# UBC-AWP/vision-sam3-yolo-lameless

Hardware: AMD Instinct MI355X
Metric: frames/sec (whole node) for YOLO+SAM3+DINOv3 feature extraction, 1080p clips (higher is better)
Workload: dtype f16; 1 GPU; BASELINE cfg#5, dense schedule: fused per-frame path on a synthetic 5 s @ 30 fps 1080p clip (150 unique BGR frames resident in HBM): YOLOv8-l detect (letterbox 384x640, NMS, scale_boxes; f16 plan) -> SAM (Hiera-B+ image encoder + FPN at 1024x1024, box-prompted mask decoder, 1080p mask + statistics + contour features) + DINOv3 ViT-L/16 embed (224x224) on EVERY frame; per-frame records packed, gathe; parallelism=one clip per GPU, 1 GPU(s), one gather per step, streams=7

## Files before the change

### include/lmx.h

```cpp
#ifndef LMX_H
#define LMX_H
#include <stdint.h>
#ifdef __cplusplus
extern "C" {
#endif

#define LMX_VERSION 100

#define LMX_OK 0
#define LMX_EINVAL (-1)
#define LMX_EHIP (-2)

typedef void* lmx_stream_t;

int lmx_version(void);
const char* lmx_last_error(void);
int lmx_device_count(void);

enum { LMX_F16 = 0, LMX_F32 = 1 };
enum { LMX_ACT_NONE = 0, LMX_ACT_SILU = 1, LMX_ACT_GELU = 2 , LMX_ACT_RELU = 3,
       LMX_ACT_SWIGLU = 4  };

typedef struct {
  const void* A;
// ... 166 lines not shown
enum { LMX_HIERA_MLP_IMG = 0, LMX_HIERA_MLP_FUSED = 1, LMX_HIERA_MLP_LAUNCHES = 2 };
typedef struct {
  int32_t H, W, Hf, Ho, Wo, Hfo, join, attn, ln1, shortcut, query, window, ln_out, mlp, emit_ln1, stage_end, keep, x16, join_out, clone;
} lmx_hiera_block_t;
int lmx_h_hiera_blocks(const lmx_hiera_config_t* config, int* n_blocks_host);
int lmx_h_hiera_plan_rows(const lmx_hiera_config_t* config, int n, const int* rows_in_host, int lowest, lmx_hiera_block_t* records_host);
int lmx_h_hiera_plan(const lmx_hiera_config_t* config, int n, int nh, int nw, int lowest, lmx_hiera_block_t* records_host, int* rows_host);

int lmx_k_add_bcast(const void* a, int a_dtype, int64_t lda, const float* b, int64_t ldb, int b_rows, void* out,
                    int out_dtype, int64_t ldo, int64_t rows, int D, lmx_stream_t stream);
int lmx_k_prompt_box(const float* boxes, int64_t ldb, float* sparse, int n, double sx, double sy, float S,
                     const float* gauss, const float* corner, int F, lmx_stream_t stream);
int lmx_k_hyper_mask(const void* up, const float* hyper, float* logits, int n, int G, int C, lmx_stream_t stream);
int lmx_k_mask_post(const float* logits, int n, int L, int T, int nh, int nw, int h, int w, uint8_t* mask,
                    int64_t* stats, float* workspace, lmx_stream_t stream);
int lmx_k_prompt_points(const float* points, const int32_t* labels, int Np, const float* boxes, int64_t ldb, float* sparse, int n,
                        double sx, double sy, float S, const float* gauss, const float* point_embed, const float* not_a_point,
                        const float* corner, int F, lmx_stream_t stream);
#define LMX_MASK_EMBED_PARAMS 4684
int lmx_k_mask_embed(const float* mask_input, const void* emb, int emb_dtype, int64_t lde, const float* params, float* keys,
                     int64_t ldk, int n, int G, lmx_stream_t stream);
int lmx_k_hyper_mask_multi(const void* up, const float* hyper, float* logits, int n, int M, int G, int C, lmx_stream_t stream);
int lmx_k_hyper_mask_multi_f32(const float* up, const float* hyper, float* logits, int n, int M, int G, int C, int act,
                               lmx_stream_t stream);
int lmx_k_mask_logits(const float* logits, int n, int L, int T, int nh, int nw, int h, int w, float* out, lmx_stream_t stream);

int lmx_k_mask_score(const float* logits, int n, int L, int T, int nh, int nw, int h, int w, double thr, double off,
                     const int32_t* idx, int64_t* out, lmx_stream_t stream);
int lmx_k_nms_boxes(const float* boxes, int64_t ldb, const float* scores, const uint8_t* valid, int n, double iou, int32_t* keep_out,
                    int32_t* count_out, void* workspace, lmx_stream_t stream);
// ... 1 lines not shown
enum { LMX_RECORD_MAX_FIELDS = 16, LMX_RECORD_MAX_MAPS = 4 };
typedef struct { const void* src; int64_t row_bytes, offset; int32_t map, n_src; } lmx_record_field_t;
int lmx_k_pack_records(const lmx_record_field_t* fields_host, int n_fields, const int32_t* const* row_maps_host, int n_maps, int64_t n_valid,
                       int64_t n_rows, int64_t stride, uint8_t* out, lmx_stream_t stream);

enum { LMX_REC_U8 = 0, LMX_REC_I32 = 1, LMX_REC_I64 = 2, LMX_REC_F32 = 3 };
enum { LMX_STREAMS_LANES = 0, LMX_STREAMS_RR = 1 };
typedef struct { char name[16]; int32_t dtype, ndim; int64_t shape[2], offset, nbytes; } lmx_record_field_layout_t;
typedef struct { int32_t n_fields, reserved; int64_t stride; lmx_record_field_layout_t fields[LMX_RECORD_MAX_FIELDS]; } lmx_record_layout_t;
int lmx_h_record_layout(int h, int w, int hidden, int max_det, int scheduled, lmx_record_layout_t* out_host);
int lmx_h_stream_plan(int n_chunks, int max_streams, int layout, int* pool_host, int* det_host, int* emb_host, int32_t* sam_host);
int lmx_h_row_map(int n, const int32_t* idx_host, int n_idx, const char* what, int32_t* map_host, int32_t* ran_host);

int64_t lmx_contour_workspace_bytes(int n, int h, int w);
int lmx_k_contour_features(const uint8_t* mask, int n, int h, int w, int64_t* out, void* workspace, lmx_stream_t stream);

int lmx_h_mask_features(const uint8_t* mask_host, int h, int w, double* out_host);

int lmx_h_iou_matrix(const double* a, int n, const double* b, int m, double* out);
int lmx_h_assign(const double* cost, int n, int m, int* row_to_col, int* col_to_row);

enum { LMX_FILT_BILINEAR = 2, LMX_FILT_BICUBIC = 3 };
int lmx_h_pil_tables(int in_size, int out_size, int filt, int32_t* bounds_host, int32_t* kk_host, int64_t cap, int* ksize_host);
int lmx_h_aa_tables(int in_size, int out_size, int filt, int32_t* bounds_host, float* kk_host, int64_t cap, int* ksize_host);
int lmx_h_identity_table(int n, int32_t* bounds_host, int32_t* kk_host);
int lmx_h_segment_cols(const int32_t* bounds_host, int n_out, int tile);

typedef struct lmx_dino lmx_dino;
enum { LMX_DINO_V2 = 0, LMX_DINO_V3 = 1 };
enum { LMX_RECIPE_PIL = 0, LMX_RECIPE_FLOAT = 1 };
// ... 216 lines not shown
```

### vision-sam3-yolo-lameless_amd/csrc/contour.hip

```cpp
#include "common.h"

namespace {

typedef unsigned long long u64;

__device__ __forceinline__ int pc(u64 v) { return __builtin_popcountll(v); }
__device__ __forceinline__ int ld(const int* p) { return __hip_atomic_load(p, __ATOMIC_RELAXED, __HIP_MEMORY_SCOPE_AGENT); }

__device__ __forceinline__ int uf_find(const int* L, int i) {
  int p = ld(L + i);
  while (p != i) {
    i = p;
    p = ld(L + i);
  }
  return i;
}

__device__ __forceinline__ void uf_union(int* L, int a, int b) {
  for (;;) {
    a = uf_find(L, a);
    b = uf_find(L, b);
    if (a == b) return;
    if (a > b) {
      const int t = a;
// ... 89 lines not shown
      cnt[wi] = c;
    }
    __syncthreads();
    int before = 0, all = 0;
#pragma unroll
    for (int i = 0; i < WPI; ++i) {
      const int c = cnt[i];
      before += i < wi ? c : 0;
      all += c;
    }
    if (leader && k < wpr) ws.wpre[ri * wpr + k] = running + before;
    running += all;
    __syncthreads();
  }
  if (threadIdx.x == 0) ws.rowbase[ri] = running;
}

__global__ __launch_bounds__(256) void run_scan_kernel(Ws ws) {
  __shared__ int part[256];
  const int img = blockIdx.x;
  int* rb = ws.rowbase + (int64_t)img * ws.h;
  int running = 2;
  for (int y0 = 0; y0 < ws.h; y0 += 256) {
    const int y = y0 + threadIdx.x;
    const int c = y < ws.h ? (rb[y] + 1) & ~1 : 0;
    part[threadIdx.x] = c;
    __syncthreads();
    for (int o = 1; o < 256; o <<= 1) {
      const int v = threadIdx.x >= o ? part[threadIdx.x - o] : 0;
      __syncthreads();
// ... 294 lines not shown
    off += bytes;
    return p;
  };
  ws.bits = reinterpret_cast<u64*>(take(words * 8));
  ws.area2 = reinterpret_cast<long long*>(take(slots * 8));
  ws.steps = reinterpret_cast<u64*>(take(slots * 8));
  ws.best = reinterpret_cast<u64*>(take((int64_t)n * 8));
  ws.box = reinterpret_cast<int*>(take(slots * 16));
  ws.L = reinterpret_cast<int*>(take((int64_t)n * ws.cap * 4));
  ws.wpre = reinterpret_cast<int*>(take(words * 4));
  ws.rowbase = reinterpret_cast<int*>(take((int64_t)n * h * 4));
  ws.count = reinterpret_cast<int*>(take((int64_t)n * 4));
  return off;
}

}

extern "C" int64_t lmx_contour_workspace_bytes(int n, int h, int w) {
  if (n <= 0 || h <= 0 || w <= 0) return 0;
  Ws ws;
  return ws_layout(ws, nullptr, n, h, w);
}

extern "C" int lmx_k_contour_features(const uint8_t* mask, int n, int h, int w, int64_t* out, void* workspace, lmx_stream_t stream) {
  LMX_REQUIRE(mask && out && workspace, "lmx_k_contour_features: null pointer");
  LMX_REQUIRE(n > 0 && h > 1 && w > 1 && (int64_t)h * w <= 0x1fffff && (int64_t)n * h < 0x7fffffffll && n <= 65535,
              "lmx_k_contour_features: n=%d h=%d w=%d (at most 2^21 - 1 pixels per mask)", n, h, w);
  LMX_REQUIRE(aligned16(workspace), "lmx_k_contour_features: workspace alignment");
  hipStream_t st = reinterpret_cast<hipStream_t>(stream);
  const int64_t npix = (int64_t)h * w;
  Ws ws;
  ws_layout(ws, reinterpret_cast<char*>(workspace), n, h, w);
  const unsigned rows = (unsigned)((int64_t)n * h), words = grid_for((int64_t)n * h * ws.wpr);
  if (w % 4 == 0 && (reinterpret_cast<uintptr_t>(mask) & 3) == 0)
    hipLaunchKernelGGL(run_bits_kernel<true>, dim3(rows), dim3(256), 0, st, mask, ws, npix);
  else
    hipLaunchKernelGGL(run_bits_kernel<false>, dim3(rows), dim3(256), 0, st, mask, ws, npix);
  hipLaunchKernelGGL(run_scan_kernel, dim3(n), dim3(256), 0, st, ws);
  hipLaunchKernelGGL(run_init_kernel, dim3(words), dim3(256), 0, st, ws, n);
  hipLaunchKernelGGL(run_union_kernel, dim3(words), dim3(256), 0, st, ws, n);
  hipLaunchKernelGGL(run_compress_kernel, dim3(words), dim3(256), 0, st, ws, n);
  hipLaunchKernelGGL(run_sum_kernel, dim3(words), dim3(256), 0, st, ws, n);
  hipLaunchKernelGGL(run_select_kernel, dim3(words), dim3(256), 0, st, ws, n);
  hipLaunchKernelGGL(contour_final_kernel, dim3((n + 63) / 64), dim3(64), 0, st, ws, reinterpret_cast<long long*>(out), n);
  return lmx_launch_check("contour_final_kernel");
}
```

### vision-sam3-yolo-lameless_amd/csrc/sam.hip

```cpp
#include "common.h"
#include "hiera_bands.h"

namespace {

inline int grid_for(int64_t total, int block = 256) {
  int64_t g = (total + block - 1) / block;
  if (g > 256 * 8) g = 256 * 8;
  if (g < 1) g = 1;
  return (int)g;
}

constexpr int P7_T = 64;
constexpr int P7_ROW = (4 * P7_T + 3) * 3;
constexpr int P7_NDW = (P7_ROW + 3 + 3) / 4 + 1;
constexpr int P7_LOADS = (7 * P7_NDW + 255) / 256;
__global__ __launch_bounds__(256) void im2col_p7_kernel(const uint8_t* __restrict__ img, const float* __restrict__ lut,
                                                        half_t* __restrict__ out, int n, int rh, int rw, int OH, int OW, int64_t ldo) {
  __shared__ half_t lut_s[768];
  __shared__ half_t st[7 * P7_ROW];
  for (int i = threadIdx.x; i < 768; i += blockDim.x) lut_s[i] = (half_t)lut[i];
  __syncthreads();
  const int tid = threadIdx.x;
  const int chunks = (int)(ldo / 8);
  const int tpp = 256 / chunks;
// ... 334 lines not shown
      maxy = red_b[k][3] > maxy ? red_b[k][3] : maxy;
    }
    if (area) {
      unsigned long long* st = stats + (int64_t)b * 8;
      atomicAdd(&st[0], area);
      atomicAdd(&st[1], sumx);
      atomicAdd(&st[2], sumy);
      atomicMin(reinterpret_cast<long long*>(&st[3]), (long long)minx);
      atomicMin(reinterpret_cast<long long*>(&st[4]), (long long)miny);
      atomicMax(reinterpret_cast<long long*>(&st[5]), (long long)maxx);
      atomicMax(reinterpret_cast<long long*>(&st[6]), (long long)maxy);
    }
  }
}

__global__ __launch_bounds__(256) void pack_bits_kernel(const uint8_t* __restrict__ src, int64_t rows, int w, int wb,
                                                        uint8_t* __restrict__ dst) {
  const int64_t total = rows * wb;
  const bool fast = (w & 7) == 0 && ((reinterpret_cast<uintptr_t>(src) & 7) == 0);
  for (int64_t i = (int64_t)blockIdx.x * blockDim.x + threadIdx.x; i < total; i += (int64_t)gridDim.x * blockDim.x) {
    const int64_t r = i / wb;
    const int c = (int)(i - r * wb);
    const uint8_t* sp = src + r * w + (int64_t)c * 8;
    unsigned long long x = 0;
    if (fast) {
      x = *reinterpret_cast<const unsigned long long*>(sp);
    } else {
      for (int e = 0; e < 8; ++e)
        if (c * 8 + e < w) x |= (unsigned long long)sp[e] << (8 * e);
    }
// ... 205 lines not shown
  else if (dbg == 5) LMX_MASK_VARIANT(5, 5)
  else if (dbg == 8) LMX_MASK_VARIANT(1, 8)
  else if (dbg == 6) LMX_MASK_VARIANT(1, 6)
  else if (dbg == 7) LMX_MASK_VARIANT(1, 7)
  else if (dbg == 1) LMX_MASK_VARIANT(1, 1)
  else if (dbg == 9) LMX_MASK_VARIANT(1, 9)
  else LMX_MASK_VARIANT(0, 0)
#undef LMX_MASK_VARIANT
#else
  hipLaunchKernelGGL(mask_mid_kernel<0>, dim3(gmid), dim3(256), 0, st, logits, workspace, n, L, T, nh, nw, su);
  hipLaunchKernelGGL(mask_post_kernel<0>, dim3(gx, n), dim3(256), 0, st, workspace, n, nh, nw, h, w, mask, su, gmid);
#endif
  return lmx_launch_check("mask_post_kernel");
}

extern "C" int lmx_k_pack_bits(const uint8_t* src, int64_t rows, int w, uint8_t* dst, lmx_stream_t stream) {
  LMX_REQUIRE(src && dst, "lmx_k_pack_bits: null pointer");
  LMX_REQUIRE(rows > 0 && w > 0, "lmx_k_pack_bits: rows=%lld w=%d", (long long)rows, w);
  const int wb = (w + 7) / 8;
  hipLaunchKernelGGL(pack_bits_kernel, dim3(grid_for(rows * wb)), dim3(256), 0, reinterpret_cast<hipStream_t>(stream), src, rows, w, wb, dst);
  return lmx_launch_check("pack_bits_kernel");
}
```

### vision-sam3-yolo-lameless_amd/csrc/sam_model.hip

```cpp
#include <math.h>
#include <string.h>

#include <map>
#include <string>
#include <tuple>
#include <vector>

#include "model_handle.h"
#include "sam_hiera_model.h"
#include "sam_image.h"
#include "sam_lanes.h"

namespace {

const int64_t MAX_BUFFER_BYTES = 0x7fffffffll;
const int DD = LMX_SAM_DEC_D, DH = LMX_SAM_DEC_HEADS, DT = LMX_SAM_OUT_TOKENS + 2;

struct Lin {
  const void* w = nullptr;
  const float *b = nullptr, *s = nullptr;
  int N = 0, K = 0;
};

struct Norm {
// ... 698 lines not shown
    LMX_TRY(upscale(W, v, nP));
    LMX_TRY(operand(queries + DD, (int64_t)T * DD, nullptr, 0, P.qc16, n, &mask_tok));
    LMX_TRY(ffn(W.hyp, mask_tok, P.hyper));
    if (exact)
      LMX_TRY(lmx_k_hyper_mask_multi_f32(static_cast<const float*>(P.u2), P.hyper, logits, n, 1, G, 32, LMX_ACT_GELU, st));
    else
      LMX_TRY(lmx_k_hyper_mask_multi(P.u2, P.hyper, logits, n, 1, G, 32, st));
    return ffn(W.iou, iou_tok, P.iou4);
  }
};

int decode_chunk(const lmx_sam* m, const Prepared& P, int precision, const void* emb, int n, int h, int w, const float* boxes, int64_t ldb, uint8_t* mask,
                 uint8_t* mask_bits, int64_t* stats, int64_t* contour, float* iou, float* lowres, hipStream_t st) {
  const LmxSamCfg& c = m->cfg;
  const int L = 4 * c.grid();
  uint8_t* mk = mask ? mask : P.mask;
  float* logits = lowres ? lowres : P.logits;
  LMX_TRY(lmx_k_prompt_box(boxes, ldb, P.sparse, n, (double)P.nw / (double)w, (double)P.nh / (double)h, (float)c.image, m->gauss, m->corner, DD / 2, st));
  LMX_HIP(hipMemcpy2DAsync(P.tokens + LMX_SAM_OUT_TOKENS * DD, (size_t)DT * DD * 4, P.sparse, (size_t)2 * DD * 4, (size_t)2 * DD * 4, (size_t)n,
                           hipMemcpyDeviceToDevice, st));
  LMX_TRY((Dec{m, P, n, precision == LMX_SAM_EXACT, st}.lowres(emb, logits)));
  LMX_TRY(lmx_k_mask_post(logits, n, L, c.image, P.nh, P.nw, h, w, mk, stats, P.post, st));
  LMX_HIP(hipMemcpy2DAsync(iou, 4, P.iou4, 16, 4, (size_t)n, hipMemcpyDeviceToDevice, st));
  if (mask_bits) LMX_TRY(lmx_k_pack_bits(mk, (int64_t)n * h, w, mask_bits, st));
  if (contour) LMX_TRY(lmx_k_contour_features(mk, n, h, w, contour, P.contour_ws, st));
  return LMX_OK;
}

int check_call(const lmx_sam* m, const char* fn, int n, int h, int w, int precision) {
  LMX_TRY(lmx_handle_on_device(m, fn));
  LMX_REQUIRE(n > 0, "%s: n = %d frames", fn, n);
  LMX_REQUIRE(h > 0 && w > 0, "%s: frame size %d x %d", fn, h, w);
  return check_precision(m, fn, precision);
}

int check_decode(const lmx_sam* m, const char* fn, const void* in, const char* in_name, int n, int h, int w, const void* boxes, int precision,
                 const void* stats, const void* contour, const void* iou) {
  LMX_TRY(check_call(m, fn, n, h, w, precision));
  LMX_REQUIRE(in != nullptr, "%s: null pointer (%s)", fn, in_name);
  LMX_REQUIRE(boxes != nullptr, "%s: null pointer (boxes)", fn);
// ... 175 lines not shown
```

### vision-sam3-yolo-lameless_amd/lmx/_lib.py

```python
import ctypes as C
import os

_HERE = os.path.dirname(os.path.abspath(__file__))
LIB_PATH = os.environ.get("LMX_LIB") or os.path.join(_HERE, "liblmx.so")


class LmxError(RuntimeError):
    pass


class GemmDesc(C.Structure):
    _fields_ = [
        ("A", C.c_void_p), ("W", C.c_void_p), ("bias", C.c_void_p), ("scale", C.c_void_p), ("res", C.c_void_p),
        ("C", C.c_void_p),
        ("lda", C.c_int64), ("ldc", C.c_int64), ("ldr", C.c_int64),
        ("M", C.c_int32), ("N", C.c_int32), ("K", C.c_int32),
        ("act", C.c_int32), ("out_dtype", C.c_int32), ("a_mode", C.c_int32),
        ("H", C.c_int32), ("W_", C.c_int32), ("Cin", C.c_int32), ("conv_stride", C.c_int32),
        ("Ho", C.c_int32), ("Wo", C.c_int32), ("res_rows", C.c_int32), ("a_rep", C.c_int32), ("split_k", C.c_int32), ("split_stride", C.c_int64),
        ("ln_out", C.c_void_p), ("ln_gamma", C.c_void_p), ("ln_beta", C.c_void_p), ("ld_ln", C.c_int64), ("ln_eps", C.c_float),
    ]


class DinoInfo(C.Structure):
# ... 196 lines not shown
    "lmx_k_im2col_u8": (_I, [_VP, _VP, _VP, _I, _I, _I, _I, _I, _I, _I, _I, _I, _I64, _VP]),
    "lmx_k_maxpool2": (_I, [_VP, _I64, _VP, _I64, _I, _I, _I, _I, _I, _VP]),
    "lmx_k_cast_f32_f16": (_I, [_VP, _I64, _VP, _I64, _I64, _I, _VP]),
    "lmx_h_hiera_band": (_I, [C.POINTER(C.c_int), C.POINTER(C.c_int), _I, _I, _I, _I, C.POINTER(C.c_int)]),
    "lmx_h_hiera_bands": (_I, [C.POINTER(C.c_int), C.POINTER(C.c_int), _I, _I, _I, _I, C.POINTER(C.c_int)]),
    "lmx_k_band_join": (_I, [_VP, _VP, _VP, _I, _I, _I, _I, _I, _I, _VP]),
    "lmx_h_hiera_blocks": (_I, [C.POINTER(HieraConfig), C.POINTER(C.c_int)]),
    "lmx_h_hiera_plan_rows": (_I, [C.POINTER(HieraConfig), _I, C.POINTER(C.c_int), _I, C.POINTER(HieraBlock)]),
    "lmx_h_hiera_plan": (_I, [C.POINTER(HieraConfig), _I, _I, _I, _I, C.POINTER(HieraBlock), C.POINTER(C.c_int)]),
    "lmx_k_add_bcast":(_I, [_VP, _I, _I64, _VP, _I64, _I, _VP, _I, _I64, _I64, _I, _VP]),
    "lmx_h_mask_features": (_I, [_VP, _I, _I, _VP]),
    "lmx_h_iou_matrix": (_I, [_VP, _I, _VP, _I, _VP]),
    "lmx_h_assign": (_I, [_VP, _I, _I, _VP, _VP]),
    "lmx_contour_workspace_bytes": (_I64, [_I, _I, _I]),
    "lmx_k_contour_features": (_I, [_VP, _I, _I, _I, _VP, _VP, _VP]),
    "lmx_k_prompt_box": (_I, [_VP, _I64, _VP, _I, _D, _D, _F, _VP, _VP, _I, _VP]),
    "lmx_k_hyper_mask": (_I, [_VP, _VP, _VP, _I, _I, _I, _VP]),
    "lmx_k_mask_post": (_I, [_VP, _I, _I, _I, _I, _I, _I, _I, _VP, _VP, _VP, _VP]),
    "lmx_k_prompt_points": (_I, [_VP, _VP, _I, _VP, _I64, _VP, _I, _D, _D, _F, _VP, _VP, _VP, _VP, _I, _VP]),
    "lmx_k_mask_embed": (_I, [_VP, _VP, _I, _I64, _VP, _VP, _I64, _I, _I, _VP]),
    "lmx_k_hyper_mask_multi": (_I, [_VP, _VP, _VP, _I, _I, _I, _I, _VP]),
    "lmx_k_hyper_mask_multi_f32": (_I, [_VP, _VP, _VP, _I, _I, _I, _I, _I, _VP]),
    "lmx_k_mask_logits": (_I, [_VP, _I, _I, _I, _I, _I, _I, _I, _VP, _VP]),
    "lmx_k_mask_score": (_I, [_VP, _I, _I, _I, _I, _I, _I, _I, _D, _D, _VP, _VP, _VP]),
    "lmx_k_nms_boxes": (_I, [_VP, _I64, _VP, _VP, _I, _D, _VP, _VP, _VP, _VP]),
    "lmx_h_pil_tables": (_I, [_I, _I, _I, _VP, _VP, _I64, C.POINTER(C.c_int)]),
    "lmx_h_aa_tables": (_I, [_I, _I, _I, _VP, _VP, _I64, C.POINTER(C.c_int)]),
    "lmx_h_identity_table": (_I, [_I, _VP, _VP]),
    "lmx_h_segment_cols": (_I, [_VP, _I, _I]),
    "lmx_dino_image_check_host": (_I, [C.c_char_p, C.POINTER(DinoInfo)]),
# ... 111 lines not shown
```

### vision-sam3-yolo-lameless_amd/lmx/kernels.py

```python
import ctypes as C
import os
import threading

import torch

from . import _lib
from ._lib import AttnDesc, GemmDesc, LmxError, check

F16, F32 = 0, 1
ACT_NONE, ACT_SILU, ACT_GELU, ACT_RELU, ACT_SWIGLU = 0, 1, 2, 3, 4
_DT = {torch.float16: F16, torch.float32: F32}


_tls = threading.local()


def _stream(dev):
    _tls.dev = dev
    return C.c_void_p(torch.cuda.current_stream(dev).cuda_stream)


def _ptr(t):
    return C.c_void_p(t.data_ptr()) if t is not None else C.c_void_p(0)

# ... 1554 lines not shown
    check(_lib.load().lmx_k_hyper_mask(_ptr(up), _ptr(hyper), _ptr(logits), n, G, C_, _stream(dev)), "lmx_k_hyper_mask")
    return logits


def mask_post(logits, T, nh, nw, h, w):
    dev = _dev(logits)
    n, L, _ = logits.shape
    mask = torch.empty((n, h, w), dtype=torch.uint8, device=logits.device)
    stats = torch.empty((n, 8), dtype=torch.int64, device=logits.device)
    ws = torch.empty((n, nh, nw), dtype=torch.float32, device=logits.device)
    check(_lib.load().lmx_k_mask_post(_ptr(logits), n, L, T, nh, nw, h, w, _ptr(mask), _ptr(stats), _ptr(ws), _stream(dev)),
          "lmx_k_mask_post")
    return mask, stats


def prompt_points(points, labels, boxes, sx, sy, S, gauss, point_embed, not_a_point, corner):
    dev = _dev(points, labels, boxes, gauss)
    Np = 0 if points is None else points.shape[1]
    if Np:
        if (points.dtype != torch.float32 or labels.dtype != torch.int32 or not points.is_contiguous() or not labels.is_contiguous()
                or points.dim() != 3 or points.shape[2] != 2 or tuple(labels.shape) != tuple(points.shape[:2])):
            raise LmxError("prompt_points: points must be contiguous f32 [n,Np,2], labels contiguous int32 [n,Np]")
    if boxes is not None and (boxes.dtype != torch.float32 or boxes.dim() != 2 or boxes.shape[1] < 4 or boxes.stride(1) != 1):
        raise LmxError("prompt_points: boxes must be f32 [n,>=4] rows")
    n = points.shape[0] if Np else boxes.shape[0]
    if boxes is not None and boxes.shape[0] != n:
        raise LmxError("prompt_points: points and boxes disagree on n")
    Fq = gauss.shape[1]
    ldb = 0 if boxes is None else (boxes.stride(0) if n > 1 else boxes.shape[1])
    out = torch.empty((n, Np + (2 if boxes is not None else 1), 2 * Fq), dtype=torch.float32, device=dev)
# ... 95 lines not shown
    ws = torch.empty((n * 5,), dtype=torch.float32, device=boxes.device)
    check(_lib.load().lmx_k_nms_boxes(_ptr(boxes), ldb, _ptr(scores), _ptr(valid), n, float(iou), _ptr(keep), _ptr(count), _ptr(ws),
                                      _stream(dev)), "lmx_k_nms_boxes")
    return keep, count


def contour_features(mask):
    dev = _dev(mask)
    if mask.dtype != torch.uint8 or mask.dim() != 3 or not mask.is_contiguous():
        raise LmxError("contour_features: mask must be contiguous uint8 [n,h,w]")
    n, h, w = mask.shape
    lib = _lib.load()
    ws = torch.empty((int(lib.lmx_contour_workspace_bytes(n, h, w)),), dtype=torch.uint8, device=mask.device)
    out = torch.empty((n, 8), dtype=torch.int64, device=mask.device)
    check(lib.lmx_k_contour_features(_ptr(mask), n, h, w, _ptr(out), _ptr(ws), _stream(dev)), "lmx_k_contour_features")
    return out


LAUNCH_TRACE = None
_raw_lib = None
RIDGE_FLOP_PER_BYTE = 2500e12 / 8e12


def _work(name, args):
    if name == "lmx_k_gemm":
        d = args[0]._obj
        M, N, Kd = d.M, d.N, d.K
        osz = 4 if d.out_dtype == F32 else 2
        a_bytes = 2 * M * (Kd // max(d.a_rep, 1))
        if d.a_mode == 1:
# ... 109 lines not shown
```

### vision-sam3-yolo-lameless_amd/lmx/pipeline.py

```python
import os

import torch

from . import dino, sam, sam_decoder, yolo
from . import kernels as K

DATA = os.path.join(os.path.dirname(os.path.abspath(__file__)), "data")


def stream_plan(n_chunks, max_streams=4, layout="lanes"):
    if layout not in ("lanes", "rr"):
        raise ValueError(f"stream layout {layout!r}: expected 'lanes' or 'rr'")
    k = max(3, min(2 + n_chunks, int(max_streams)))
    if layout == "rr":
        return k, 0, 1, [(2 + j) % k for j in range(n_chunks)]
    return k, 0, 1, [2 + j % (k - 2) for j in range(n_chunks)]


class FusedExtractor:
    def __init__(self, device="cuda", yolo_scale="l", weight_seeds=(7, 5, 3), yolo_bn=None):
        from . import weights

        self.device = torch.device(device)
        self.serial = bool(os.environ.get("LMX_SERIAL"))
# ... 51 lines not shown
            out["ran_det"].index_fill_(0, di, 1)
            if keep_byte_masks:
                out["mask"] = torch.zeros((n, h, w), dtype=torch.uint8, device=dev)
                out["mask"].index_copy_(0, di, part["mask"])
        if ei.numel():
            out["embedding"].index_copy_(0, ei, part["embedding"])
            out["ran_emb"].index_fill_(0, ei, 1)
        return out

    def _step_dense(self, frames, conf, sam_chunk, keep_byte_masks, emb_frames=None, precision=None):
        n, h, w, _ = frames.shape
        emb_frames = frames if emb_frames is None else emb_frames
        rhw = sam.resize_longest_side(h, w, self.sam.cfg.image)
        main = torch.cuda.current_stream(self.device)
        chunks = list(range(0, n, sam_chunk))
        if self.serial:
            det_stream, emb_stream, sam_streams = main, main, [main] * len(chunks)
        else:
            n_pool, di, ei, si = stream_plan(max(1, len(chunks)), self.max_streams, self.stream_layout)
            pool = self._streams(n_pool)
            det_stream, emb_stream, sam_streams = pool[di], pool[ei], [pool[j] for j in si][:len(chunks)]
            for st in pool:
                st.wait_stream(main)
        empty = n == 0
        with torch.cuda.stream(det_stream):
            if empty:
                z = torch.zeros
                boxes, scores, cls, counts = (z((0, 300, 4), device=self.device), z((0, 300), device=self.device),
                                              z((0, 300), dtype=torch.int32, device=self.device), z((0,), dtype=torch.int32, device=self.device))
            else:
                boxes, scores, cls, src, counts = self.yolo.detect(frames, conf=conf, precision=precision)
            det_done = torch.cuda.Event()
            det_done.record(det_stream)
        with torch.cuda.stream(emb_stream):
            emb = (self.dino.embed_frames(emb_frames) if emb_frames.shape[0]
                   else torch.zeros((0, self.dino.cfg.hidden), dtype=torch.float32, device=self.device))
        masks, stats, ious, conts = [], [], [], []
        for i, st in zip(chunks, sam_streams):
            with torch.cuda.stream(st):
                enc = self.sam.encode(frames[i:i + sam_chunk], precision=precision, outputs="embedding")
                e2 = enc["fpn"][2]
                st.wait_event(det_done)
                d = self.decoder.predict(e2.view(-1, e2.shape[-1]), boxes[i:i + sam_chunk, 0, :], (h, w), rhw, precision=precision)
                conts.append(K.contour_features(d["mask"]))
            masks.append(d["mask"])
            stats.append(d["stats"])
            ious.append(d["iou"])
        for st in set(sam_streams + [det_stream, emb_stream]):
            if st is not main:
                main.wait_stream(st)
        if empty:
            mask = torch.zeros((0, h, w), dtype=torch.uint8, device=self.device)
            out = dict(boxes=boxes, scores=scores, cls=cls, counts=counts, embedding=emb,
                       mask_bits=torch.zeros((0, h, (w + 7) // 8), dtype=torch.uint8, device=self.device),
                       mask_stats=torch.zeros((0, 8), dtype=torch.int64, device=self.device),
                       mask_contour=torch.zeros((0, 8), dtype=torch.int64, device=self.device),
                       mask_iou=torch.zeros((0,), dtype=torch.float32, device=self.device))
        else:
            cat = (lambda ts: ts[0] if len(ts) == 1 else torch.cat(ts, 0))
            mask = cat(masks)
            out = dict(boxes=boxes, scores=scores, cls=cls, counts=counts, embedding=emb, mask_bits=K.pack_bits(mask),
                       mask_stats=cat(stats), mask_contour=cat(conts), mask_iou=cat(ious))
        if keep_byte_masks:
            out["mask"] = mask
        return out
```

### vision-sam3-yolo-lameless_amd/lmx/sam_decoder.py

```python
import math

import numpy as np
import torch

from . import kernels as K

D = 256
HEADS = 8


def param_spec():
    s = {}
    s["shared_image_embedding.positional_embedding"] = ((2, 128), "tok")
    s["prompt_encoder.shared_embedding.positional_embedding"] = ((2, 128), "tok")
    s["prompt_encoder.no_mask_embed.weight"] = ((1, D), "tok")
    for i in range(4):
        s[f"prompt_encoder.point_embed.{i}.weight"] = ((1, D), "tok")
    s["prompt_encoder.not_a_point_embed.weight"] = ((1, D), "tok")
    s["mask_decoder.iou_token.weight"] = ((1, D), "tok")
    s["mask_decoder.mask_tokens.weight"] = ((4, D), "tok")

    def attn(p, inner):
        for n_ in ("q_proj", "k_proj", "v_proj"):
            s[p + n_ + ".weight"] = ((inner, D), "w")
# ... 253 lines not shown
            hs = [self._ffn(P, f"mask_decoder.output_hypernetworks_mlps.{m}.", P.operand(q3[:, 1 + m].contiguous())) for m in sel]
            return hs[0][:, None] if len(hs) == 1 else torch.stack(hs, 1)

        logits = P.upscale_and_mask(v_, hyper, n)
        iou = self._ffn(P, "mask_decoder.iou_prediction_head.", iou_tok)
        return (logits[:, 0], iou[:, 0]) if masks is None else (logits, iou)

    def predict(self, emb, boxes, frame_hw, resized_hw, precision=None):
        h, w = frame_hw
        nh, nw = resized_hw
        sparse = K.prompt_box(boxes, nw / w, nh / h, float(self.S), self.gauss, self.corner)
        logits, iou = self.lowres(emb, sparse, precision=precision)
        mask, stats = K.mask_post(logits, self.S, nh, nw, h, w)
        return dict(mask=mask, stats=stats, iou=iou, lowres=logits)

    def decode_lowres(self, emb, frame_hw, resized_hw, points=None, labels=None, boxes=None, mask_input=None, multimask=False,
                      precision=None, input_frame=False):
        h, w = frame_hw
        nh, nw = resized_hw
        if points is None and boxes is None:
            raise ValueError("decode needs points (with labels) or boxes")
        if (points is None) != (labels is None):
            raise ValueError("points and labels go together")
        self._plan(precision)
        sx, sy = (1.0, 1.0) if input_frame else (nw / w, nh / h)
        sparse = K.prompt_points(points, labels, boxes, sx, sy, float(self.S), self.gauss, self.point_embed, self.not_a_point,
                                 self.corner)
        n, P = sparse.shape[0], self.G * self.G
        if emb.shape[0] == P and n > 1:
            emb = emb.repeat(n, 1)
# ... 28 lines not shown
```

Before: 815.6 frames/s.

## Fuse mask upsample with bit packing and feed contour labels from packed words

Adds a mask post-processing kernel that upsamples the low-res logits and thresholds them. It writes packed row bits and 64-bit words directly via wave ballots, optionally skipping the 1080p byte mask entirely. The contour-feature pass now starts from those words, with a wave-level scan replacing the byte-to-bit conversion kernel. This removes the full-resolution byte mask write, the separate pack_bits pass and the contour byte read, at the cost of a more complex kernel with atomics for the statistics.

```diff
diff --git a/include/lmx.h b/include/lmx.h
--- a/include/lmx.h
+++ b/include/lmx.h
@@ -204,6 +204,8 @@
 int lmx_k_hyper_mask(const void* up, const float* hyper, float* logits, int n, int G, int C, lmx_stream_t stream);
 int lmx_k_mask_post(const float* logits, int n, int L, int T, int nh, int nw, int h, int w, uint8_t* mask,
                     int64_t* stats, float* workspace, lmx_stream_t stream);
+int lmx_k_mask_post_bits(const float* logits, int n, int L, int T, int nh, int nw, int h, int w, uint8_t* mask, uint8_t* bits,
+                         uint64_t* words, int64_t* stats, float* workspace, lmx_stream_t stream);
 int lmx_k_prompt_points(const float* points, const int32_t* labels, int Np, const float* boxes, int64_t ldb, float* sparse, int n,
                         double sx, double sy, float S, const float* gauss, const float* point_embed, const float* not_a_point,
                         const float* corner, int F, lmx_stream_t stream);
@@ -235,6 +237,8 @@
 
 int64_t lmx_contour_workspace_bytes(int n, int h, int w);
 int lmx_k_contour_features(const uint8_t* mask, int n, int h, int w, int64_t* out, void* workspace, lmx_stream_t stream);
+int lmx_contour_workspace_bits(int n, int h, int w, int64_t* offset_host, int64_t* bytes_host);
+int lmx_k_contour_features_words(const uint64_t* words, int n, int h, int w, int64_t* out, void* workspace, lmx_stream_t stream);
 
 int lmx_h_mask_features(const uint8_t* mask_host, int h, int w, double* out_host);
 
diff --git a/vision-sam3-yolo-lameless_amd/csrc/contour.hip b/vision-sam3-yolo-lameless_amd/csrc/contour.hip
--- a/vision-sam3-yolo-lameless_amd/csrc/contour.hip
+++ b/vision-sam3-yolo-lameless_amd/csrc/contour.hip
@@ -127,6 +127,33 @@
     __syncthreads();
   }
   if (threadIdx.x == 0) ws.rowbase[ri] = running;
+}
+
+__global__ __launch_bounds__(256) void run_words_kernel(Ws ws, int64_t rows) {
+  const int lane = threadIdx.x & 63;
+  const int64_t ri = (int64_t)blockIdx.x * 4 + (threadIdx.x >> 6);
+  if (ri >= rows) return;
+  const int wpr = ws.wpr;
+  const u64* b = ws.bits + ri * wpr;
+  int running = 0;
+  for (int k0 = 0; k0 < wpr; k0 += 64) {
+    const int k = k0 + lane;
+    int c = 0;
+    if (k < wpr) {
+      const u64 word = b[k];
+      const u64 prev = k > 0 ? b[k - 1] >> 63 : (~word & 1);
+      c = pc((word ^ ((word << 1) | prev)) & valid_bits(ws.w, wpr, k));
+    }
+    int inc = c;
+#pragma unroll
+    for (int o = 1; o < 64; o <<= 1) {
+      const int v = __shfl_up(inc, o, 64);
+      if (lane >= o) inc += v;
+    }
+    if (k < wpr) ws.wpre[ri * wpr + k] = running + inc - c;
+    running += __shfl(inc, 63, 64);
+  }
+  if (lane == 0) ws.rowbase[ri] = running;
 }
 
 __global__ __launch_bounds__(256) void run_scan_kernel(Ws ws) {
@@ -451,6 +478,18 @@
   return off;
 }
 
+inline int run_labels(const Ws& ws, int n, int64_t* out, hipStream_t st) {
+  const unsigned words = grid_for((int64_t)n * ws.h * ws.wpr);
+  hipLaunchKernelGGL(run_scan_kernel, dim3(n), dim3(256), 0, st, ws);
+  hipLaunchKernelGGL(run_init_kernel, dim3(words), dim3(256), 0, st, ws, n);
+  hipLaunchKernelGGL(run_union_kernel, dim3(words), dim3(256), 0, st, ws, n);
+  hipLaunchKernelGGL(run_compress_kernel, dim3(words), dim3(256), 0, st, ws, n);
+  hipLaunchKernelGGL(run_sum_kernel, dim3(words), dim3(256), 0, st, ws, n);
+  hipLaunchKernelGGL(run_select_kernel, dim3(words), dim3(256), 0, st, ws, n);
+  hipLaunchKernelGGL(contour_final_kernel, dim3((n + 63) / 64), dim3(64), 0, st, ws, reinterpret_cast<long long*>(out), n);
+  return lmx_launch_check("contour_final_kernel");
+}
+
 }
 
 extern "C" int64_t lmx_contour_workspace_bytes(int n, int h, int w) {
@@ -468,17 +507,35 @@
   const int64_t npix = (int64_t)h * w;
   Ws ws;
   ws_layout(ws, reinterpret_cast<char*>(workspace), n, h, w);
-  const unsigned rows = (unsigned)((int64_t)n * h), words = grid_for((int64_t)n * h * ws.wpr);
+  const unsigned rows = (unsigned)((int64_t)n * h);
   if (w % 4 == 0 && (reinterpret_cast<uintptr_t>(mask) & 3) == 0)
     hipLaunchKernelGGL(run_bits_kernel<true>, dim3(rows), dim3(256), 0, st, mask, ws, npix);
   else
     hipLaunchKernelGGL(run_bits_kernel<false>, dim3(rows), dim3(256), 0, st, mask, ws, npix);
-  hipLaunchKernelGGL(run_scan_kernel, dim3(n), dim3(256), 0, st, ws);
-  hipLaunchKernelGGL(run_init_kernel, dim3(words), dim3(256), 0, st, ws, n);
-  hipLaunchKernelGGL(run_union_kernel, dim3(words), dim3(256), 0, st, ws, n);
-  hipLaunchKernelGGL(run_compress_kernel, dim3(words), dim3(256), 0, st, ws, n);
-  hipLaunchKernelGGL(run_sum_kernel, dim3(words), dim3(256), 0, st, ws, n);
-  hipLaunchKernelGGL(run_select_kernel, dim3(words), dim3(256), 0, st, ws, n);
-  hipLaunchKernelGGL(contour_final_kernel, dim3((n + 63) / 64), dim3(64), 0, st, ws, reinterpret_cast<long long*>(out), n);
-  return lmx_launch_check("contour_final_kernel");
-}
+  return run_labels(ws, n, out, st);
+}
+
+extern "C" int lmx_contour_workspace_bits(int n, int h, int w, int64_t* offset_host, int64_t* bytes_host) {
+  LMX_REQUIRE(offset_host && bytes_host, "lmx_contour_workspace_bits: null pointer");
+  LMX_REQUIRE(n > 0 && h > 0 && w > 0, "lmx_contour_workspace_bits: n=%d h=%d w=%d", n, h, w);
+  Ws ws;
+  ws_layout(ws, nullptr, n, h, w);
+  *offset_host = (int64_t)reinterpret_cast<intptr_t>(ws.bits);
+  *bytes_host = (int64_t)n * h * ws.wpr * 8;
+  return LMX_OK;
+}
+
+extern "C" int lmx_k_contour_features_words(const uint64_t* words, int n, int h, int w, int64_t* out, void* workspace, lmx_stream_t stream) {
+  LMX_REQUIRE(words && out && workspace, "lmx_k_contour_features_words: null pointer");
+  LMX_REQUIRE(n > 0 && h > 1 && w > 1 && (int64_t)h * w <= 0x1fffff && (int64_t)n * h < 0x7fffffffll && n <= 65535,
+              "lmx_k_contour_features_words: n=%d h=%d w=%d (at most 2^21 - 1 pixels per mask)", n, h, w);
+  LMX_REQUIRE(aligned16(workspace), "lmx_k_contour_features_words: workspace alignment");
+  LMX_REQUIRE((reinterpret_cast<uintptr_t>(words) & 7) == 0, "lmx_k_contour_features_words: words must be 8-byte aligned");
+  hipStream_t st = reinterpret_cast<hipStream_t>(stream);
+  Ws ws;
+  ws_layout(ws, reinterpret_cast<char*>(workspace), n, h, w);
+  ws.bits = const_cast<u64*>(reinterpret_cast<const u64*>(words));
+  const int64_t rows = (int64_t)n * h;
+  hipLaunchKernelGGL(run_words_kernel, dim3((unsigned)((rows + 3) / 4)), dim3(256), 0, st, ws, rows);
+  return run_labels(ws, n, out, st);
+}
diff --git a/vision-sam3-yolo-lameless_amd/csrc/sam.hip b/vision-sam3-yolo-lameless_amd/csrc/sam.hip
--- a/vision-sam3-yolo-lameless_amd/csrc/sam.hip
+++ b/vision-sam3-yolo-lameless_amd/csrc/sam.hip
@@ -372,6 +372,127 @@
   }
 }
 
+constexpr int MPB_ROWS = 8;
+constexpr int MPB_MAX_RSEG = 1 << 15;
+
+template <bool MASK>
+__global__ __launch_bounds__(256) void mask_post_bits_kernel(const float* __restrict__ mid, int nh, int nw, int h, int w, int rseg,
+                                                             uint8_t* __restrict__ mask, uint8_t* __restrict__ bits,
+                                                             unsigned long long* __restrict__ words,
+                                                             unsigned long long* __restrict__ stats) {
+  typedef unsigned long long u64;
+  const int b = blockIdx.y;
+  const int lane = threadIdx.x & 63;
+  const int wv = __builtin_amdgcn_readfirstlane((int)(threadIdx.x >> 6));
+  const int wpr = (w + 63) / 64, wb = (w + 7) / 8;
+  const int tiles = wpr * ((h + rseg - 1) / rseg);
+  const float* md = mid + (int64_t)b * nh * nw;
+  const float sy = (float)nh / (float)h, sx = (float)nw / (float)w;
+  const int64_t row0 = (int64_t)b * h;
+  u64 area = 0, sumx = 0, sumy = 0;
+  int minx = 0x7fffffff, miny = 0x7fffffff, maxx = -1, maxy = -1;
+  for (int t = blockIdx.x * 4 + wv; t < tiles; t += gridDim.x * 4) {
+    const int k = t % wpr, seg = t / wpr;
+    const int x = 64 * k + lane;
+    const bool inx = x < w;
+    int X0, X1;
+    float lx;
+    bil_idx(sx, inx ? x : w - 1, nw, X0, X1, lx);
+    const float lx0 = 1.f - lx;
+    const int ys = seg * rseg, y1 = ys + rseg < h ? ys + rseg : h;
+    unsigned cnt = 0, rel = 0;
+    int ty0 = 0x7fffffff, ty1 = -1;
+    for (int yg = ys; yg < y1; yg += MPB_ROWS) {
+      float a00[MPB_ROWS], a01[MPB_ROWS], a10[MPB_ROWS], a11[MPB_ROWS], ly[MPB_ROWS];
+#pragma unroll
+      for (int r = 0; r < MPB_ROWS; ++r) {
+        const int y = yg + r < y1 ? yg + r : y1 - 1;
+        int Y0, Y1;
+        bil_idx(sy, y, nh, Y0, Y1, ly[r]);
+        const float* r0 = md + (int64_t)Y0 * nw;
+        const float* r1 = md + (int64_t)Y1 * nw;
+        a00[r] = r0[X0], a01[r] = r0[X1], a10[r] = r1[X0], a11[r] = r1[X1];
+      }
+      __builtin_amdgcn_sched_barrier(0);
+      u64 mine = 0;
+#pragma unroll
+      for (int r = 0; r < MPB_ROWS; ++r) {
+        const int y = yg + r;
+        const bool live = y < y1;
+        const float t0 = lx0 * a00[r] + lx * a01[r];
+        const float t1 = lx0 * a10[r] + lx * a11[r];
+        const float v = (1.f - ly[r]) * t0 + ly[r] * t1;
+        const bool on = (v > 0.0f) & inx & live;
+        const u64 word = __ballot(on);
+        mine = lane == r ? word : mine;
+        cnt += on ? 1u : 0u;
+        rel += on ? (unsigned)(y - ys) : 0u;
+        if (MASK && inx && live) mask[(row0 + y) * w + x] = on ? 1 : 0;
+        const bool any = word != 0;
+        ty0 = any && y < ty0 ? y : ty0;
+        ty1 = any ? y : ty1;
+      }
+      if (words && lane < MPB_ROWS && yg + lane < y1) words[(row0 + yg + lane) * wpr + k] = mine;
+      if (bits) {
+        const int r = lane >> 3, bb = lane & 7;
+        const u64 wr = __shfl(mine, r, 64);
+        if (yg + r < y1 && 8 * k + bb < wb) bits[(row0 + yg + r) * wb + 8 * k + bb] = __builtin_bitreverse8((uint8_t)(wr >> (8 * bb)));
+      }
+    }
+    const u64 have = __ballot(cnt != 0);
+    if (have) {
+      u64 a = cnt, qx = (u64)(unsigned)x * cnt, qy = (u64)rel + (u64)(unsigned)ys * cnt;
+#pragma unroll
+      for (int o = 32; o > 0; o >>= 1) {
+        a += __shfl_xor(a, o, 64);
+        qx += __shfl_xor(qx, o, 64);
+        qy += __shfl_xor(qy, o, 64);
+      }
+      area += a;
+      sumx += qx;
+      sumy += qy;
+      const int lo = 64 * k + __ffsll((long long)have) - 1, hi = 64 * k + 63 - (int)__clzll((long long)have);
+      minx = lo < minx ? lo : minx;
+      maxx = hi > maxx ? hi : maxx;
+      miny = ty0 < miny ? ty0 : miny;
+      maxy = ty1 > maxy ? ty1 : maxy;
+    }
+  }
+  __shared__ u64 red_s[4][3];
+  __shared__ int red_b[4][4];
+  if (lane == 0) {
+    red_s[wv][0] = area;
+    red_s[wv][1] = sumx;
+    red_s[wv][2] = sumy;
+    red_b[wv][0] = minx;
+    red_b[wv][1] = miny;
+    red_b[wv][2] = maxx;
+    red_b[wv][3] = maxy;
+  }
+  __syncthreads();
+  if (threadIdx.x == 0) {
+    for (int i = 1; i < 4; ++i) {
+      area += red_s[i][0];
+      sumx += red_s[i][1];
+      sumy += red_s[i][2];
+      minx = red_b[i][0] < minx ? red_b[i][0] : minx;
+      miny = red_b[i][1] < miny ? red_b[i][1] : miny;
+      maxx = red_b[i][2] > maxx ? red_b[i][2] : maxx;
+      maxy = red_b[i][3] > maxy ? red_b[i][3] : maxy;
+    }
+    if (area) {
+      u64* st = stats + (int64_t)b * 8;
+      atomicAdd(&st[0], area);
+      atomicAdd(&st[1], sumx);
+      atomicAdd(&st[2], sumy);
+      atomicMin(reinterpret_cast<long long*>(&st[3]), (long long)minx);
+      atomicMin(reinterpret_cast<long long*>(&st[4]), (long long)miny);
+      atomicMax(reinterpret_cast<long long*>(&st[5]), (long long)maxx);
+      atomicMax(reinterpret_cast<long long*>(&st[6]), (long long)maxy);
+    }
+  }
+}
+
 __global__ __launch_bounds__(256) void pack_bits_kernel(const uint8_t* __restrict__ src, int64_t rows, int w, int wb,
                                                         uint8_t* __restrict__ dst) {
   const int64_t total = rows * wb;
@@ -607,6 +728,35 @@
   return lmx_launch_check("mask_post_kernel");
 }
 
+extern "C" int lmx_k_mask_post_bits(const float* logits, int n, int L, int T, int nh, int nw, int h, int w, uint8_t* mask, uint8_t* bits,
+                                    uint64_t* words, int64_t* stats, float* workspace, lmx_stream_t stream) {
+  LMX_REQUIRE(logits && stats && workspace, "lmx_k_mask_post_bits: null pointer");
+  LMX_REQUIRE(mask || bits || words, "lmx_k_mask_post_bits: one of mask, bits and words must be asked for");
+  LMX_REQUIRE(n > 0 && L > 0 && T >= L && nh > 0 && nw > 0 && nh <= T && nw <= T && h > 0 && w > 0 &&
+                  (int64_t)h * ((w + 3) / 4) < 0x7fffffffll - 96 * 256 && n <= 65535, "lmx_k_mask_post_bits: geometry");
+  LMX_REQUIRE((reinterpret_cast<uintptr_t>(words) & 7) == 0, "lmx_k_mask_post_bits: words must be 8-byte aligned");
+  hipStream_t st = reinterpret_cast<hipStream_t>(stream);
+  hipLaunchKernelGGL(mask_stats_init_kernel, dim3((n * 8 + 255) / 256), dim3(256), 0, st, reinterpret_cast<long long*>(stats), n);
+  const int64_t wpr = (w + 63) / 64;
+  int64_t waves = wpr * ((h + 15) / 16);
+  if (waves > 96 * 4) waves = 96 * 4;
+  int64_t segs = waves / wpr;
+  if (segs < 1) segs = 1;
+  int rseg = (int)((h + segs - 1) / segs);
+  if (rseg > MPB_MAX_RSEG) rseg = MPB_MAX_RSEG;
+  const int64_t tiles = wpr * ((h + rseg - 1) / rseg);
+  int gx = (int)((tiles + 3) / 4);
+  if (gx > 96) gx = 96;
+  unsigned long long* su = reinterpret_cast<unsigned long long*>(stats);
+  hipLaunchKernelGGL(mask_mid_kernel<0>, dim3(grid_for((int64_t)n * nh * nw)), dim3(256), 0, st, logits, workspace, n, L, T, nh, nw, su);
+  unsigned long long* wd = reinterpret_cast<unsigned long long*>(words);
+  if (mask)
+    hipLaunchKernelGGL(mask_post_bits_kernel<true>, dim3(gx, n), dim3(256), 0, st, workspace, nh, nw, h, w, rseg, mask, bits, wd, su);
+  else
+    hipLaunchKernelGGL(mask_post_bits_kernel<false>, dim3(gx, n), dim3(256), 0, st, workspace, nh, nw, h, w, rseg, mask, bits, wd, su);
+  return lmx_launch_check("mask_post_bits_kernel");
+}
+
 extern "C" int lmx_k_pack_bits(const uint8_t* src, int64_t rows, int w, uint8_t* dst, lmx_stream_t stream) {
   LMX_REQUIRE(src && dst, "lmx_k_pack_bits: null pointer");
   LMX_REQUIRE(rows > 0 && w > 0, "lmx_k_pack_bits: rows=%lld w=%d", (long long)rows, w);
diff --git a/vision-sam3-yolo-lameless_amd/csrc/sam_model.hip b/vision-sam3-yolo-lameless_amd/csrc/sam_model.hip
--- a/vision-sam3-yolo-lameless_amd/csrc/sam_model.hip
+++ b/vision-sam3-yolo-lameless_amd/csrc/sam_model.hip
@@ -736,16 +736,21 @@
                  uint8_t* mask_bits, int64_t* stats, int64_t* contour, float* iou, float* lowres, hipStream_t st) {
   const LmxSamCfg& c = m->cfg;
   const int L = 4 * c.grid();
-  uint8_t* mk = mask ? mask : P.mask;
   float* logits = lowres ? lowres : P.logits;
+  uint64_t* words = nullptr;
+  if (contour) {
+    int64_t off = 0, bytes = 0;
+    LMX_TRY(lmx_contour_workspace_bits(n, h, w, &off, &bytes));
+    words = reinterpret_cast<uint64_t*>(static_cast<char*>(P.contour_ws) + off);
+  }
   LMX_TRY(lmx_k_prompt_box(boxes, ldb, P.sparse, n, (double)P.nw / (double)w, (double)P.nh / (double)h, (float)c.image, m->gauss, m->corner, DD / 2, st));
   LMX_HIP(hipMemcpy2DAsync(P.tokens + LMX_SAM_OUT_TOKENS * DD, (size_t)DT * DD * 4, P.sparse, (size_t)2 * DD * 4, (size_t)2 * DD * 4, (size_t)n,
                            hipMemcpyDeviceToDevice, st));
   LMX_TRY((Dec{m, P, n, precision == LMX_SAM_EXACT, st}.lowres(emb, logits)));
-  LMX_TRY(lmx_k_mask_post(logits, n, L, c.image, P.nh, P.nw, h, w, mk, stats, P.post, st));
+  uint8_t* mk = mask || mask_bits || words ? mask : P.mask;
+  LMX_TRY(lmx_k_mask_post_bits(logits, n, L, c.image, P.nh, P.nw, h, w, mk, mask_bits, words, stats, P.post, st));
   LMX_HIP(hipMemcpy2DAsync(iou, 4, P.iou4, 16, 4, (size_t)n, hipMemcpyDeviceToDevice, st));
-  if (mask_bits) LMX_TRY(lmx_k_pack_bits(mk, (int64_t)n * h, w, mask_bits, st));
-  if (contour) LMX_TRY(lmx_k_contour_features(mk, n, h, w, contour, P.contour_ws, st));
+  if (contour) LMX_TRY(lmx_k_contour_features_words(words, n, h, w, contour, P.contour_ws, st));
   return LMX_OK;
 }
 
diff --git a/vision-sam3-yolo-lameless_amd/lmx/_lib.py b/vision-sam3-yolo-lameless_amd/lmx/_lib.py
--- a/vision-sam3-yolo-lameless_amd/lmx/_lib.py
+++ b/vision-sam3-yolo-lameless_amd/lmx/_lib.py
@@ -234,6 +234,9 @@
     "lmx_h_assign": (_I, [_VP, _I, _I, _VP, _VP]),
     "lmx_contour_workspace_bytes": (_I64, [_I, _I, _I]),
     "lmx_k_contour_features": (_I, [_VP, _I, _I, _I, _VP, _VP, _VP]),
+    "lmx_contour_workspace_bits": (_I, [_I, _I, _I, C.POINTER(C.c_int64), C.POINTER(C.c_int64)]),
+    "lmx_k_contour_features_words": (_I, [_VP, _I, _I, _I, _VP, _VP, _VP]),
+    "lmx_k_mask_post_bits": (_I, [_VP, _I, _I, _I, _I, _I, _I, _I, _VP, _VP, _VP, _VP, _VP, _VP]),
     "lmx_k_prompt_box": (_I, [_VP, _I64, _VP, _I, _D, _D, _F, _VP, _VP, _I, _VP]),
     "lmx_k_hyper_mask": (_I, [_VP, _VP, _VP, _I, _I, _I, _VP]),
     "lmx_k_mask_post": (_I, [_VP, _I, _I, _I, _I, _I, _I, _I, _VP, _VP, _VP, _VP]),
diff --git a/vision-sam3-yolo-lameless_amd/lmx/kernels.py b/vision-sam3-yolo-lameless_amd/lmx/kernels.py
--- a/vision-sam3-yolo-lameless_amd/lmx/kernels.py
+++ b/vision-sam3-yolo-lameless_amd/lmx/kernels.py
@@ -1592,6 +1592,31 @@
     return mask, stats
 
 
+def mask_post_bits(logits, T, nh, nw, h, w, mask=False, bits=True, words=None):
+    dev = _dev(logits, words, *(t for t in (mask, bits) if isinstance(t, torch.Tensor)))
+    n, L, _ = logits.shape
+
+    def out(t, shape, dtype, what):
+        if t is None or t is False:
+            return None
+        if t is True:
+            return torch.empty(shape, dtype=dtype, device=logits.device)
+        if t.dtype != dtype or tuple(t.shape) != shape or not t.is_contiguous():
+            raise LmxError(f"mask_post_bits: {what} must be contiguous {dtype} {list(shape)}")
+        return t
+
+    mask = out(mask, (n, h, w), torch.uint8, "mask")
+    bits = out(bits, (n, h, (w + 7) // 8), torch.uint8, "bits")
+    words = out(words, (n, h, (w + 63) // 64), torch.int64, "words")
+    if mask is None and bits is None and words is None:
+        raise LmxError("mask_post_bits: one of mask, bits and words must be asked for")
+    stats = torch.empty((n, 8), dtype=torch.int64, device=logits.device)
+    ws = torch.empty((n, nh, nw), dtype=torch.float32, device=logits.device)
+    check(_lib.load().lmx_k_mask_post_bits(_ptr(logits), n, L, T, nh, nw, h, w, _ptr(mask), _ptr(bits), _ptr(words), _ptr(stats), _ptr(ws),
+                                           _stream(dev)), "lmx_k_mask_post_bits")
+    return mask, bits, stats
+
+
 def prompt_points(points, labels, boxes, sx, sy, S, gauss, point_embed, not_a_point, corner):
     dev = _dev(points, labels, boxes, gauss)
     Np = 0 if points is None else points.shape[1]
@@ -1717,6 +1742,29 @@
     ws = torch.empty((int(lib.lmx_contour_workspace_bytes(n, h, w)),), dtype=torch.uint8, device=mask.device)
     out = torch.empty((n, 8), dtype=torch.int64, device=mask.device)
     check(lib.lmx_k_contour_features(_ptr(mask), n, h, w, _ptr(out), _ptr(ws), _stream(dev)), "lmx_k_contour_features")
+    return out
+
+
+def contour_workspace(n, h, w, device):
+    lib = _lib.load()
+    off, size = C.c_int64(0), C.c_int64(0)
+    check(lib.lmx_contour_workspace_bits(n, h, w, C.byref(off), C.byref(size)), "lmx_contour_workspace_bits")
+    ws = torch.empty((int(lib.lmx_contour_workspace_bytes(n, h, w)),), dtype=torch.uint8, device=device)
+    return ws, ws[off.value:off.value + size.value].view(torch.int64).view(n, h, (w + 63) // 64)
+
+
+def contour_features_words(words, w, ws=None):
+    dev = _dev(words, ws)
+    if words.dtype != torch.int64 or words.dim() != 3 or not words.is_contiguous() or words.shape[2] != (w + 63) // 64:
+        raise LmxError("contour_features_words: words must be contiguous int64 [n,h,ceil(w/64)]")
+    n, h, _ = words.shape
+    lib = _lib.load()
+    if ws is None:
+        ws = torch.empty((int(lib.lmx_contour_workspace_bytes(n, h, w)),), dtype=torch.uint8, device=words.device)
+    elif ws.dtype != torch.uint8 or not ws.is_contiguous() or ws.numel() < int(lib.lmx_contour_workspace_bytes(n, h, w)):
+        raise LmxError("contour_features_words: workspace smaller than lmx_contour_workspace_bytes(n, h, w)")
+    out = torch.empty((n, 8), dtype=torch.int64, device=words.device)
+    check(lib.lmx_k_contour_features_words(_ptr(words), n, h, w, _ptr(out), _ptr(ws), _stream(dev)), "lmx_k_contour_features_words")
     return out
 
 
diff --git a/vision-sam3-yolo-lameless_amd/lmx/pipeline.py b/vision-sam3-yolo-lameless_amd/lmx/pipeline.py
--- a/vision-sam3-yolo-lameless_amd/lmx/pipeline.py
+++ b/vision-sam3-yolo-lameless_amd/lmx/pipeline.py
@@ -3,7 +3,6 @@
 import torch
 
 from . import dino, sam, sam_decoder, yolo
-from . import kernels as K
 
 DATA = os.path.join(os.path.dirname(os.path.abspath(__file__)), "data")
 
@@ -89,6 +88,8 @@
         rhw = sam.resize_longest_side(h, w, self.sam.cfg.image)
         main = torch.cuda.current_stream(self.device)
         chunks = list(range(0, n, sam_chunk))
+        bits = torch.empty((n, h, (w + 7) // 8), dtype=torch.uint8, device=self.device)
+        mask = torch.empty((n, h, w), dtype=torch.uint8, device=self.device) if keep_byte_masks else None
         if self.serial:
             det_stream, emb_stream, sam_streams = main, main, [main] * len(chunks)
         else:
@@ -110,22 +111,21 @@
         with torch.cuda.stream(emb_stream):
             emb = (self.dino.embed_frames(emb_frames) if emb_frames.shape[0]
                    else torch.zeros((0, self.dino.cfg.hidden), dtype=torch.float32, device=self.device))
-        masks, stats, ious, conts = [], [], [], []
+        stats, ious, conts = [], [], []
         for i, st in zip(chunks, sam_streams):
             with torch.cuda.stream(st):
                 enc = self.sam.encode(frames[i:i + sam_chunk], precision=precision, outputs="embedding")
                 e2 = enc["fpn"][2]
                 st.wait_event(det_done)
-                d = self.decoder.predict(e2.view(-1, e2.shape[-1]), boxes[i:i + sam_chunk, 0, :], (h, w), rhw, precision=precision)
-                conts.append(K.contour_features(d["mask"]))
-            masks.append(d["mask"])
+                d = self.decoder.predict_bits(e2.view(-1, e2.shape[-1]), boxes[i:i + sam_chunk, 0, :], (h, w), rhw, precision=precision,
+                                              bits=bits[i:i + sam_chunk], byte_mask=mask[i:i + sam_chunk] if keep_byte_masks else False)
+            conts.append(d["contour"])
             stats.append(d["stats"])
             ious.append(d["iou"])
         for st in set(sam_streams + [det_stream, emb_stream]):
             if st is not main:
                 main.wait_stream(st)
         if empty:
-            mask = torch.zeros((0, h, w), dtype=torch.uint8, device=self.device)
             out = dict(boxes=boxes, scores=scores, cls=cls, counts=counts, embedding=emb,
                        mask_bits=torch.zeros((0, h, (w + 7) // 8), dtype=torch.uint8, device=self.device),
                        mask_stats=torch.zeros((0, 8), dtype=torch.int64, device=self.device),
@@ -133,8 +133,7 @@
                        mask_iou=torch.zeros((0,), dtype=torch.float32, device=self.device))
         else:
             cat = (lambda ts: ts[0] if len(ts) == 1 else torch.cat(ts, 0))
-            mask = cat(masks)
-            out = dict(boxes=boxes, scores=scores, cls=cls, counts=counts, embedding=emb, mask_bits=K.pack_bits(mask),
+            out = dict(boxes=boxes, scores=scores, cls=cls, counts=counts, embedding=emb, mask_bits=bits,
                        mask_stats=cat(stats), mask_contour=cat(conts), mask_iou=cat(ious))
         if keep_byte_masks:
             out["mask"] = mask
diff --git a/vision-sam3-yolo-lameless_amd/lmx/sam_decoder.py b/vision-sam3-yolo-lameless_amd/lmx/sam_decoder.py
--- a/vision-sam3-yolo-lameless_amd/lmx/sam_decoder.py
+++ b/vision-sam3-yolo-lameless_amd/lmx/sam_decoder.py
@@ -291,6 +291,18 @@
         mask, stats = K.mask_post(logits, self.S, nh, nw, h, w)
         return dict(mask=mask, stats=stats, iou=iou, lowres=logits)
 
+    def predict_bits(self, emb, boxes, frame_hw, resized_hw, precision=None, bits=True, byte_mask=False):
+        h, w = frame_hw
+        nh, nw = resized_hw
+        sparse = K.prompt_box(boxes, nw / w, nh / h, float(self.S), self.gauss, self.corner)
+        logits, iou = self.lowres(emb, sparse, precision=precision)
+        ws, words = K.contour_workspace(logits.shape[0], h, w, logits.device)
+        mask, bits, stats = K.mask_post_bits(logits, self.S, nh, nw, h, w, mask=byte_mask, bits=bits, words=words)
+        out = dict(mask_bits=bits, stats=stats, contour=K.contour_features_words(words, w, ws), iou=iou, lowres=logits)
+        if mask is not None:
+            out["mask"] = mask
+        return out
+
     def decode_lowres(self, emb, frame_hw, resized_hw, points=None, labels=None, boxes=None, mask_input=None, multimask=False,
                       precision=None, input_frame=False):
         h, w = frame_hw
```

After: 821.5 frames/s, median of 6. No clear change (+0.7%).
